# finmath/finmath-lib-cuda-extensions

Measured on AMD Instinct MI355X. Metric: Monte-Carlo path-ops/sec (fused RandomVariable stream), higher is better.
Workload: dtype f32

## Files before the change

finmath-lib-cuda-extensions_amd/host/lmm.hpp:

```cpp
#pragma once
#include <algorithm>
#include <chrono>
#include <cmath>
#include <cstdio>
#include <atomic>
#include <thread>
#include <cstdlib>
#include <functional>
#include <string>
#include <vector>

#include "random_variable.hpp"

namespace fmhost { namespace lmm {


inline const std::vector<double>& atmNormalVolatilities() {
    static const std::vector<double> v = {
        0.00151, 0.00169, 0.0021, 0.00248, 0.00291, 0.00329, 0.00365, 0.004, 0.00437, 0.00466, 0.00527, 0.00571,
        0.00604, 0.00625, 0.0016, 0.00174, 0.00217, 0.00264, 0.00314, 0.00355, 0.00398, 0.00433, 0.00469,
        0.00493, 0.00569, 0.00607, 0.00627, 0.00645, 0.00182, 0.00204, 0.00238, 0.00286, 0.00339, 0.00384,
        0.00424, 0.00456, 0.00488, 0.0052, 0.0059, 0.00623, 0.0064, 0.00654, 0.00205, 0.00235, 0.00272, 0.0032,
        0.00368, 0.00406, 0.00447, 0.00484, 0.00515, 0.00544, 0.00602, 0.00629, 0.0064, 0.00646, 0.00279,
        0.00319, 0.0036, 0.00396, 0.00436, 0.00469, 0.00503, 0.0053, 0.00557, 0.00582, 0.00616, 0.00628,
// ... 71 lines not shown
                for (int p = 0; p < s.numberOfPeriods; ++p) {
                    const double d = curve.df(s.swapTenor[p + 1]);
                    floating += curve.forward(s.swapTenor[p], 0.5) * 0.5 * d; annuity += 0.5 * d;
                }
                s.swaprate = floating / annuity; s.annuity = annuity;
                s.targetVolatility = vols[e * atmTenorYears().size() + k];
                swaptions.push_back(std::move(s));
            }
    }
    int numberOfLibors() const { return timeDiscretization.getNumberOfTimeSteps(); }
};

struct VolatilityModel {
    std::vector<double> grid{ 0.0, 1.0, 2.0, 5.0, 10.0, 20.0, 30.0, 40.0 };
    std::vector<double> parameter = std::vector<double>(64, 0.50 / 100);
    int bin(double x) const { int k = 0; while (k < 7 && grid[(size_t)k] < x - 1e-12) ++k; return k; }
    int parameterIndex(double time, double maturity) const { return bin(time) * 8 + bin(maturity - time); }
    double volatility(double time, double maturity) const { return maturity <= time + 1e-12 ? 0.0 : parameter[(size_t)parameterIndex(time, maturity)]; }
    std::vector<int> activeParameters(const Market& m) const {
        std::vector<char> used(64, 0);
        const auto& td = m.timeDiscretization;
        for (int i = 0; i < td.getNumberOfTimeSteps(); ++i)
            for (int j = i + 1; j < m.numberOfLibors(); ++j) used[(size_t)parameterIndex(td.getTime(i), td.getTime(j))] = 1;
        std::vector<int> idx;
        for (int k = 0; k < 64; ++k) if (used[(size_t)k]) idx.push_back(k);
        return idx;
    }
};


struct Simulation {
    std::vector<std::vector<RV>> libor;
    std::vector<RV> numeraire;
};

struct Backend {
    const RandomVariableFactory* factory = nullptr;
    const BrownianMotion* brownianMotion = nullptr;
    std::function<void()> flush = [] {};
    std::function<void(bool)> hold = [](bool) {};
    std::function<long long()> launches = [] { return 0LL; };
    std::function<std::vector<double>(const std::vector<RV>&)> averages = [](const std::vector<RV>& v) {
        std::vector<double> a; for (const RV& x : v) a.push_back(x->getAverage()); return a; };
    std::function<std::function<std::vector<double>()>(const std::vector<RV>&)> averagesAsync;
    bool expectationsRunPending = false;
    std::function<void(const std::vector<RV>&)> valuesNotNeeded;
    int chunk = 7;
    int stepsPerLaunch = 4;
    std::function<std::vector<std::vector<RV>>(const std::vector<RV>& roots, const std::vector<RV>& leafFrom, const std::vector<std::vector<RV>>& leafTo,
                                               const std::vector<std::vector<double>>* scalars)> clone;
    std::function<std::vector<double>(const std::vector<RV>& roots)> recordedScalars;
    int jacobianBatch = 1;
    bool keepAllStates = false;
    int threads = 1;
};

inline std::vector<Simulation> simulateMany(const Market& m, const std::vector<const VolatilityModel*>& vols, const Backend& be, int lastTimeIndex,
                                            const std::vector<char>* keep = nullptr) {
    const auto& td = m.timeDiscretization;
    const int n = m.numberOfLibors();
    const double delta = m.dt;
    const size_t K = vols.size();
    std::vector<Simulation> sims(K);
    for (Simulation& sim : sims) {
        sim.libor.resize((size_t)lastTimeIndex + 1);
        sim.numeraire.resize((size_t)lastTimeIndex + 1);
        sim.libor[0].resize((size_t)n);
        for (int j = 0; j < n; ++j) sim.libor[0][(size_t)j] = be.factory->createRandomVariable(0.0, m.curve.forward(td.getTime(j), delta));
        sim.numeraire[0] = be.factory->createRandomVariable(0.0, 1.0);
    }
    std::vector<RV> factorSum(K);
    const int S = std::max(1, be.stepsPerLaunch);
    static int cloneChecks = 0;
    for (int i0 = 0; i0 < lastTimeIndex;) {
        int i1 = std::min(i0 + S, lastTimeIndex);
        static const bool endAtKept = std::getenv("FMHIP_LMM_GROUPS_END_AT_KEPT") && std::getenv("FMHIP_LMM_GROUPS_END_AT_KEPT")[0] == '1';
        if (keep && endAtKept) for (int s2 = i0 + 1; s2 < i1; ++s2) if ((*keep)[(size_t)s2]) { i1 = s2; break; }
        const bool cloning = K > 1 && S > 1 && keep && be.clone && i0 >= 2;
        const size_t Krec = cloning ? 1 : K;
        if (S > 1) be.hold(true);
        for (int i = i0; i < i1; ++i) {
            const double t = td.getTime(i), dt = td.getTimeStep(i);
            const RV dW = be.brownianMotion->getBrownianIncrement(i, 0);
            for (size_t k = 0; k < Krec; ++k) {
                auto& cur = sims[k].libor[(size_t)i];
                auto& nxt = sims[k].libor[(size_t)i + 1];
                nxt.resize((size_t)n);
                for (int j = 0; j <= i && j < n; ++j) nxt[(size_t)j] = cur[(size_t)j];
                factorSum[k] = nullptr;
            }
            for (int j0 = i + 1; j0 < n; j0 += be.chunk) {
                const int j1 = std::min(n, j0 + be.chunk);
                for (size_t k = 0; k < Krec; ++k) {
                    auto& cur = sims[k].libor[(size_t)i];
                    auto& nxt = sims[k].libor[(size_t)i + 1];
                    for (int j = j0; j < j1; ++j) {
                        const double lambda = vols[k]->volatility(t, td.getTime(j));
                        const RV& L = cur[(size_t)j];
                        const RV transform = be.factory->createRandomVariable(lambda * delta)->discount(L, delta);
                        factorSum[k] = factorSum[k] ? factorSum[k]->add(transform) : transform;
                        const RV drift = factorSum[k]->mult(lambda);
                        nxt[(size_t)j] = L->addProduct(drift, dt)->addProduct(dW, lambda);
                    }
                }
                if (S == 1 && j1 - j0 == be.chunk) be.flush();
            }
            for (size_t k = 0; k < Krec; ++k)
                sims[k].numeraire[(size_t)i + 1] = sims[k].numeraire[(size_t)i]->accrue(sims[k].libor[(size_t)i][(size_t)i], delta);
            for (size_t k = 0; k < Krec; ++k) factorSum[k] = nullptr;
        }
        if (cloning) {
            std::vector<RV> roots, leafFrom;
            for (int j = i0 + 1; j < n; ++j) roots.push_back(sims[0].libor[(size_t)i1][(size_t)j]);
            for (int i = i0; i < i1; ++i) roots.push_back(sims[0].numeraire[(size_t)i + 1]);
            for (int s2 = i0 + 1; s2 < i1; ++s2)
                if (!keep || (*keep)[(size_t)s2]) for (int j = s2; j < n; ++j) roots.push_back(sims[0].libor[(size_t)s2][(size_t)j]);
            for (int j = i0; j < n; ++j) leafFrom.push_back(sims[0].libor[(size_t)i0][(size_t)j]);
            leafFrom.push_back(sims[0].numeraire[(size_t)i0]);
            auto scalarsOf = [&](const VolatilityModel& vol) {
                std::vector<double> sc;
                for (int i = i0; i < i1; ++i) {
                    const double t = td.getTime(i), dt = td.getTimeStep(i);
                    for (int j = i + 1; j < n; ++j) {
                        const double lambda = vol.volatility(t, td.getTime(j));
                        sc.push_back(delta); sc.push_back(1.0); sc.push_back(lambda * delta); sc.push_back(lambda); sc.push_back(dt); sc.push_back(lambda);
                    }
                    sc.push_back(delta);
                }
                return sc;
            };
            if (cloneChecks < 64 && be.recordedScalars) {
                ++cloneChecks;
                if (be.recordedScalars(roots) != scalarsOf(*vols[0])) throw std::runtime_error("lmm: the scalar list of the replicated Euler steps does not match the recording");
            }
            std::vector<std::vector<RV>> leafTo(K - 1);
            std::vector<std::vector<double>> scalars(K - 1);
            for (size_t k = 1; k < K; ++k) {
                for (int j = i0; j < n; ++j) leafTo[k - 1].push_back(sims[k].libor[(size_t)i0][(size_t)j]);
                leafTo[k - 1].push_back(sims[k].numeraire[(size_t)i0]);
                scalars[k - 1] = scalarsOf(*vols[k]);
            }
            const std::vector<std::vector<RV>> copies = be.clone(roots, leafFrom, leafTo, &scalars);
            for (size_t k = 1; k < K; ++k) {
                auto& nxt = sims[k].libor[(size_t)i1];
                nxt.resize((size_t)n);
                for (int j = 0; j <= i0 && j < n; ++j) nxt[(size_t)j] = sims[k].libor[(size_t)i0][(size_t)j];
                size_t r = 0;
                for (int j = i0 + 1; j < n; ++j) nxt[(size_t)j] = copies[k - 1][r++];
                for (int i = i0; i < i1; ++i) sims[k].numeraire[(size_t)i + 1] = copies[k - 1][r++];
                for (int s2 = i0 + 1; s2 < i1; ++s2)
                    if (!keep || (*keep)[(size_t)s2]) { auto& mid = sims[k].libor[(size_t)s2]; mid.resize((size_t)n); for (int j = s2; j < n; ++j) mid[(size_t)j] = copies[k - 1][r++]; }
            }
        }
        if (keep)
            for (int i = i0; i < i1; ++i)
                if (!(*keep)[(size_t)i])
                    for (size_t k = 0; k < K; ++k) { sims[k].libor[(size_t)i].clear(); sims[k].libor[(size_t)i].shrink_to_fit(); }
        if (S > 1) be.hold(false);
        be.flush();
        i0 = i1;
    }
    return sims;
}

inline Simulation simulate(const Market& m, const VolatilityModel& vol, const Backend& be, int lastTimeIndex) {
    return std::move(simulateMany(m, { &vol }, be, lastTimeIndex)[0]);
}

inline RV swaptionValue(const Market& m, const Simulation& sim, const Swaption& s) {
    const auto& td = m.timeDiscretization;
    const int exerciseIndex = td.getTimeIndex(s.exercise);
    RV value;
    for (int p = s.numberOfPeriods - 1; p >= 0; --p) {
        const int j = td.getTimeIndex(s.swapTenor[(size_t)p]);
        const RV& libor = sim.libor[(size_t)exerciseIndex][(size_t)j];
        const RV payoff = libor->sub(s.swaprate)->mult(s.swapPeriodLength);
        value = (value ? value->add(payoff) : payoff)->discount(libor, s.swapPeriodLength);
    }
    return value->floor(0.0)->div(sim.numeraire[(size_t)exerciseIndex]);
}
inline double bachelierAtmImpliedVolatility(double optionValue, double optionMaturity, double annuity) {
    return optionValue * std::sqrt(2.0 * 3.14159265358979323846) / (annuity * std::sqrt(optionMaturity));
}

struct Valuation { std::vector<double> modelVolatility; double seconds_simulation = 0, seconds_valuation = 0; long long launches_simulation = 0, launches_valuation = 0; };

struct PendingValuations {
    std::vector<std::function<std::vector<double>()>> expectations;
    std::vector<Valuation> out;
};

inline std::vector<Valuation> evaluateManyFinish(const Market& m, PendingValuations& p) {
    for (size_t k = 0; k < p.out.size(); ++k) {
        const std::vector<double> optionValues = p.expectations[k]();
        for (size_t q = 0; q < m.swaptions.size(); ++q)
            p.out[k].modelVolatility.push_back(bachelierAtmImpliedVolatility(optionValues[q], m.swaptions[q].exercise, m.swaptions[q].annuity));
    }
    return std::move(p.out);
}

inline PendingValuations evaluateManyBegin(const Market& m, const std::vector<const VolatilityModel*>& vols, const Backend& be) {
    using clk = std::chrono::steady_clock;
    const size_t K = vols.size();
    PendingValuations pending;
    std::vector<Valuation>& out = pending.out;
    out.resize(K);
    int lastIndex = 0;
    for (const Swaption& s : m.swaptions) lastIndex = std::max(lastIndex, m.timeDiscretization.getTimeIndex(s.exercise));
    const auto t0 = clk::now();
    const long long l0 = be.launches();
    std::vector<char> keep((size_t)lastIndex + 1, 0);
    for (const Swaption& s : m.swaptions) keep[(size_t)m.timeDiscretization.getTimeIndex(s.exercise)] = 1;
    const std::vector<Simulation> sims = simulateMany(m, vols, be, lastIndex, be.keepAllStates ? nullptr : &keep);
    const auto t1 = clk::now();
    const long long l1 = be.launches();
    std::vector<std::vector<RV>> values(K);
    if (K > 1 && be.clone) {
        be.hold(true);
        values[0].reserve(m.swaptions.size());
        for (const Swaption& s : m.swaptions) values[0].push_back(swaptionValue(m, sims[0], s));
        std::vector<RV> leafFrom;
        std::vector<std::vector<RV>> leafTo(K - 1);
        for (int e = 0; e <= lastIndex; ++e) {
            if (!keep[(size_t)e]) continue;
            for (size_t k = 0; k < K; ++k) {
                std::vector<RV>& dst = k == 0 ? leafFrom : leafTo[k - 1];
                for (int j = e; j < m.numberOfLibors(); ++j) dst.push_back(sims[k].libor[(size_t)e][(size_t)j]);
                dst.push_back(sims[k].numeraire[(size_t)e]);
            }
        }
        const std::vector<std::vector<RV>> copies = be.clone(values[0], leafFrom, leafTo, nullptr);
        for (size_t k = 1; k < K; ++k) values[k] = copies[k - 1];
        be.hold(false);
        if (!(be.averagesAsync && be.expectationsRunPending)) be.flush();
    } else
    for (size_t k = 0; k < K; ++k) {
        be.hold(true);
        values[k].reserve(m.swaptions.size());
        for (const Swaption& s : m.swaptions) values[k].push_back(swaptionValue(m, sims[k], s));
        be.hold(false);
        if (!(be.averagesAsync && be.expectationsRunPending)) be.flush();
    }
    if (be.valuesNotNeeded) for (size_t k = 0; k < K; ++k) be.valuesNotNeeded(values[k]);
    for (size_t k = 0; k < K; ++k) {
        if (be.averagesAsync) pending.expectations.push_back(be.averagesAsync(values[k]));
        else { const std::vector<double> now = be.averages(values[k]); pending.expectations.push_back([now] { return now; }); }
    }
    const auto t2 = clk::now();
    for (size_t k = 0; k < K; ++k) {
        out[k].launches_simulation = (l1 - l0) / (long long)K; out[k].launches_valuation = (be.launches() - l1) / (long long)K;
        out[k].seconds_simulation = std::chrono::duration<double>(t1 - t0).count() / (double)K;
        out[k].seconds_valuation = std::chrono::duration<double>(t2 - t1).count() / (double)K;
    }
    return pending;
}

inline std::vector<Valuation> evaluateMany(const Market& m, const std::vector<const VolatilityModel*>& vols, const Backend& be) {
    PendingValuations p = evaluateManyBegin(m, vols, be);
    return evaluateManyFinish(m, p);
}

inline Valuation evaluate(const Market& m, const VolatilityModel& vol, const Backend& be) {
    return std::move(evaluateMany(m, { &vol }, be)[0]);
}


struct CalibrationResult {
    VolatilityModel model; int iterations = 0, evaluations = 0;
    double meanDeviation = 0, rmsDeviation = 0, initialRms = 0, seconds = 0, seconds_simulation = 0, seconds_valuation = 0;
    std::vector<double> modelVolatility;
};

inline bool solveSymmetric(std::vector<double> A, std::vector<double> b, int n, std::vector<double>& x) {
    for (int c = 0; c < n; ++c) {
        int piv = c;
        for (int r = c + 1; r < n; ++r) if (std::fabs(A[(size_t)r * n + c]) > std::fabs(A[(size_t)piv * n + c])) piv = r;
        if (std::fabs(A[(size_t)piv * n + c]) < 1e-300) return false;
        if (piv != c) { for (int k = 0; k < n; ++k) std::swap(A[(size_t)c * n + k], A[(size_t)piv * n + k]); std::swap(b[(size_t)c], b[(size_t)piv]); }
        for (int r = c + 1; r < n; ++r) {
            const double f = A[(size_t)r * n + c] / A[(size_t)c * n + c];
            for (int k = c; k < n; ++k) A[(size_t)r * n + k] -= f * A[(size_t)c * n + k];
            b[(size_t)r] -= f * b[(size_t)c];
        }
    }
    x.assign((size_t)n, 0.0);
    for (int r = n - 1; r >= 0; --r) { double s = b[(size_t)r]; for (int k = r + 1; k < n; ++k) s -= A[(size_t)r * n + k] * x[(size_t)k]; x[(size_t)r] = s / A[(size_t)r * n + r]; }
    return true;
}

inline CalibrationResult calibrate(const Market& m, const Backend& be, int maxIterations = 200, double accuracy = 1e-7,
                                   double lambda = 0.1, double parameterStep = 1e-4, bool verbose = false) {
    using clk = std::chrono::steady_clock;
    const auto start = clk::now();
    CalibrationResult res;
    VolatilityModel vol;
    const std::vector<int> active = vol.activeParameters(m);
    const int np = (int)active.size(), nr = (int)m.swaptions.size();
    auto residuals = [&](const VolatilityModel& v, std::vector<double>& r, std::vector<double>* modelVols) {
        const Valuation val = evaluate(m, v, be);
        res.evaluations++; res.seconds_simulation += val.seconds_simulation; res.seconds_valuation += val.seconds_valuation;
        r.resize((size_t)nr);
        for (int k = 0; k < nr; ++k) r[(size_t)k] = val.modelVolatility[(size_t)k] - m.swaptions[(size_t)k].targetVolatility;
        if (modelVols) *modelVols = val.modelVolatility;
    };
    auto sumsq = [](const std::vector<double>& r) { double s = 0; for (double x : r) s += x * x; return s; };
    std::vector<double> r, rTrial, modelVols;
    residuals(vol, r, &modelVols);
    double err = sumsq(r);
    res.initialRms = std::sqrt(err / nr);
    for (int it = 0; it < maxIterations; ++it) {
        std::vector<double> J((size_t)nr * np);
        struct InFlight { int a0 = 0, a1 = 0; std::vector<VolatilityModel> bumped; PendingValuations pending; bool valid = false; };
        auto collect = [&](InFlight& f) {
            if (!f.valid) return;
            const std::vector<Valuation> vals = evaluateManyFinish(m, f.pending);
            for (int a = f.a0; a < f.a1; ++a) {
                const Valuation& val = vals[(size_t)(a - f.a0)];
                res.evaluations++; res.seconds_simulation += val.seconds_simulation; res.seconds_valuation += val.seconds_valuation;
                for (int k = 0; k < nr; ++k) J[(size_t)k * np + a] = (val.modelVolatility[(size_t)k] - m.swaptions[(size_t)k].targetVolatility - r[(size_t)k]) / parameterStep;
            }
            f.valid = false;
        };
        if (be.threads > 1 && be.jacobianBatch <= 1) {
            const auto tj0 = clk::now();
            std::vector<Valuation> column((size_t)np);
            std::vector<std::string> failures((size_t)be.threads);
            std::atomic<int> next{ 0 };
            std::vector<std::thread> pool;
            for (int t = 0; t < be.threads; ++t)
                pool.emplace_back([&, t] {
                    try {
                        for (int a = next.fetch_add(1); a < np; a = next.fetch_add(1)) {
                            VolatilityModel bumped = vol;
                            bumped.parameter[(size_t)active[(size_t)a]] += parameterStep;
                            column[(size_t)a] = evaluate(m, bumped, be);
                        }
                    } catch (const std::exception& e) { failures[(size_t)t] = e.what(); }
                });
            for (std::thread& th : pool) th.join();
            if (std::getenv("FMHIP_LMM_TIMELINE")) std::fprintf(stderr, "[lmm timeline] iteration %d: %d columns on %d threads, %.3f … %.3f ms\n", it, np, be.threads, std::chrono::duration<double, std::milli>(tj0 - start).count(), std::chrono::duration<double, std::milli>(clk::now() - start).count());
            for (const std::string& f : failures) if (!f.empty()) throw std::runtime_error("a Jacobian column failed: " + f);
            for (int a = 0; a < np; ++a) {
                const Valuation& val = column[(size_t)a];
                res.evaluations++; res.seconds_simulation += val.seconds_simulation; res.seconds_valuation += val.seconds_valuation;
                for (int k = 0; k < nr; ++k) J[(size_t)k * np + a] = (val.modelVolatility[(size_t)k] - m.swaptions[(size_t)k].targetVolatility - r[(size_t)k]) / parameterStep;
            }
        } else {
        InFlight previous;
        for (int a0 = 0; a0 < np; a0 += std::max(1, be.jacobianBatch)) {
            const int a1 = std::min(np, a0 + std::max(1, be.jacobianBatch));
            InFlight current;
            current.a0 = a0; current.a1 = a1;
            current.bumped.assign((size_t)(a1 - a0), vol);
            std::vector<const VolatilityModel*> ptrs;
            for (int a = a0; a < a1; ++a) { current.bumped[(size_t)(a - a0)].parameter[(size_t)active[(size_t)a]] += parameterStep; ptrs.push_back(&current.bumped[(size_t)(a - a0)]); }
            static const bool timeline = std::getenv("FMHIP_LMM_TIMELINE") != nullptr;
            const auto tb0 = clk::now();
            try { current.pending = evaluateManyBegin(m, ptrs, be); current.valid = true; }
            catch (const std::exception& e) {
                if (ptrs.size() == 1 || std::string(e.what()).find("allocation") == std::string::npos) throw;
                if (verbose) std::fprintf(stderr, "  batch of %zu bumps does not fit (%s): evaluating them one at a time\n", ptrs.size(), e.what());
                be.flush();
                collect(previous);
                for (int a = a0; a < a1; ++a) {
                    const Valuation val = evaluate(m, current.bumped[(size_t)(a - a0)], be);
                    res.evaluations++; res.seconds_simulation += val.seconds_simulation; res.seconds_valuation += val.seconds_valuation;
                    for (int k = 0; k < nr; ++k) J[(size_t)k * np + a] = (val.modelVolatility[(size_t)k] - m.swaptions[(size_t)k].targetVolatility - r[(size_t)k]) / parameterStep;
                }
                continue;
            }
            const auto tb1 = clk::now();
            collect(previous);
            if (timeline) std::fprintf(stderr, "[lmm timeline] iteration %d batch from %d: begin %.3f … %.3f ms, previous collected at %.3f ms\n", it, a0,
                                       std::chrono::duration<double, std::milli>(tb0 - start).count(), std::chrono::duration<double, std::milli>(tb1 - start).count(),
                                       std::chrono::duration<double, std::milli>(clk::now() - start).count());
            previous = std::move(current);
        }
        collect(previous);
        }
        std::vector<double> JtJ((size_t)np * np, 0.0), Jtr((size_t)np, 0.0);
        for (int a = 0; a < np; ++a) {
            for (int b = 0; b < np; ++b) { double s = 0; for (int k = 0; k < nr; ++k) s += J[(size_t)k * np + a] * J[(size_t)k * np + b]; JtJ[(size_t)a * np + b] = s; }
            double s = 0; for (int k = 0; k < nr; ++k) s += J[(size_t)k * np + a] * r[(size_t)k]; Jtr[(size_t)a] = -s;
        }
        bool improved = false;
        for (int attempt = 0; attempt < 8 && !improved; ++attempt) {
            std::vector<double> A = JtJ, step;
            for (int a = 0; a < np; ++a) A[(size_t)a * np + a] += lambda * std::max(JtJ[(size_t)a * np + a], 1e-12);
            if (!solveSymmetric(A, Jtr, np, step)) { lambda *= 4; continue; }
            VolatilityModel v = vol;
            for (int a = 0; a < np; ++a) v.parameter[(size_t)active[(size_t)a]] += step[(size_t)a];
            std::vector<double> mv;
            const auto tt0 = clk::now();
            residuals(v, rTrial, &mv);
            static const bool timeline2 = std::getenv("FMHIP_LMM_TIMELINE") != nullptr;
            if (timeline2) std::fprintf(stderr, "[lmm timeline] iteration %d trial %d: %.3f … %.3f ms\n", it, attempt, std::chrono::duration<double, std::milli>(tt0 - start).count(),
                                        std::chrono::duration<double, std::milli>(clk::now() - start).count());
            const double e = sumsq(rTrial);
            if (e < err) { improved = true; const double rel = (err - e) / err; vol = v; r = rTrial; err = e; modelVols = mv; lambda = std::max(lambda / 3.0, 1e-9); if (rel < accuracy) it = maxIterations; }
            else lambda *= 4.0;
        }
        res.iterations++;
        if (verbose) std::fprintf(stderr, "  LM iteration %d: rms %.6e  lambda %.3g  evaluations %d\n", res.iterations, std::sqrt(err / nr), lambda, res.evaluations);
        if (!improved || std::sqrt(err / nr) < accuracy) break;
    }
    res.model = vol; res.modelVolatility = modelVols;
    double sum = 0; for (double x : r) sum += x;
    res.meanDeviation = sum / nr; res.rmsDeviation = std::sqrt(err / nr);
    res.seconds = std::chrono::duration<double>(clk::now() - start).count();
    return res;
}

}}
```

finmath-lib-cuda-extensions_amd/host/lmm_hip_main.cpp:

```cpp
#include <fstream>
#include <thread>
#include <csignal>
#include <execinfo.h>
#include <unistd.h>
#include <rccl/rccl.h>
#include "lmm_main_common.hpp"
#include "hip_backend.hpp"
using namespace fmhost;

static void ncclCheck(ncclResult_t r, const char* what) {
    if (r != ncclSuccess) throw std::runtime_error(std::string(what) + ": " + ncclGetErrorString(r));
}

static void fatalSignal(int sig) {
    void* frames[64];
    const int n = backtrace(frames, 64);
    const char msg[] = "lmm_hip: fatal signal, call stack:\n";
    (void)!write(2, msg, sizeof msg - 1);
    backtrace_symbols_fd(frames, n, 2);
    signal(sig, SIG_DFL);
    raise(sig);
}

int main(int argc, char** argv) {
    if (std::getenv("FMHIP_BACKTRACE")) { signal(SIGABRT, fatalSignal); signal(SIGSEGV, fatalSignal); signal(SIGBUS, fatalSignal); }
    const lmm::Options o = lmm::parseOptions(argc, argv);
    try {
        if (!o.devices.empty()) check(fmhip_init_devices(o.devices.data(), (int)o.devices.size()));
        else check(fmhip_init(-1));
        check(fmhip_set_fusion(1, nullptr));
        RandomVariableHipFactory factory;
        lmm::Market m;
        const int64_t pathOffset = o.pathOffset + (int64_t)o.rank * o.paths;
        BrownianMotionHip philox(m.timeDiscretization, 1, o.paths, o.seed, pathOffset);
        BrownianMotionFromMersenneRandomNumbers mersenne(m.timeDiscretization, 1, o.paths, (int)o.seed, &factory);
        if (o.brownian == "mersenne" && o.world > 1) throw std::runtime_error("--brownian mersenne is a sequential stream: not available with --world > 1 (mersenne-device is)");
        BrownianMotionFromMersenneRandomNumbersHip mersenneDevice(m.timeDiscretization, 1, o.paths, (int)o.seed, pathOffset);
        lmm::Backend be = makeHipBackend(&factory, (o.brownian == "mersenne") ? static_cast<const BrownianMotion*>(&mersenne)
                                                 : (o.brownian == "mersenne-device") ? static_cast<const BrownianMotion*>(&mersenneDevice) : &philox,
                                         o.chunk, o.stepsPerLaunch, o.jacobianBatch);

        if (o.finmathLike) {
            be.flush = [] {}; be.hold = [](bool) {}; be.clone = nullptr; be.recordedScalars = nullptr; be.averagesAsync = nullptr; be.expectationsRunPending = false;
            be.averages = [](const std::vector<RV>& v) { std::vector<double> a; for (const RV& x : v) a.push_back(x->getAverage()); return a; };
            be.jacobianBatch = 1; be.stepsPerLaunch = 1; be.chunk = 1 << 30; be.keepAllStates = true;
            if (o.threads > 1) {
                if (!o.devices.empty() || o.world > 1) throw std::runtime_error("--threads: one device, one process");
                check(fmhip_set_thread_engines(1, nullptr));
                be.threads = o.threads;
            }
        } else if (o.threads > 1) throw std::runtime_error("--threads belongs to --finmath-like (the native driver batches its Jacobian columns instead)");
        if (o.releaseLagMs > 0.0 || o.releaseLagBytes > 0) ReleaseLag::instance().start(o.releaseLagMs, (size_t)o.releaseLagBytes);
        ncclComm_t comm = nullptr;
        std::vector<std::pair<double*, hipEvent_t>> sparePinned;
        fmhip_vec sums = 0;
        long long collectives = 0;
        double collective_seconds = 0.0;
        if (o.world > 1 || !o.ncclIdFile.empty()) {
            if (o.ncclIdFile.empty()) throw std::runtime_error("--world needs --nccl-id-file");
            struct IdFile { uint64_t magic, nonce; ncclUniqueId id; } rec{};
            const uint64_t MAGIC = 0x464d4e43434c4944ull;
            if (o.rank == 0) {
                std::remove(o.ncclIdFile.c_str());
                rec.magic = MAGIC; rec.nonce = (uint64_t)o.ncclNonce;
                ncclCheck(ncclGetUniqueId(&rec.id), "ncclGetUniqueId");
                { std::ofstream f(o.ncclIdFile + ".tmp", std::ios::binary); f.write((const char*)&rec, sizeof rec); }
                std::rename((o.ncclIdFile + ".tmp").c_str(), o.ncclIdFile.c_str());
            } else {
                for (int tries = 0; ; ++tries) {
                    std::ifstream f(o.ncclIdFile, std::ios::binary);
                    if (f && f.read((char*)&rec, sizeof rec) && f.gcount() == (std::streamsize)sizeof rec && rec.magic == MAGIC && rec.nonce == (uint64_t)o.ncclNonce) break;
                    if (tries > 6000) throw std::runtime_error("timed out waiting for " + o.ncclIdFile);
                    std::this_thread::sleep_for(std::chrono::milliseconds(10));
                }
            }
            const ncclUniqueId id = rec.id;
            ncclCheck(ncclCommInitRank(&comm, o.world, id, o.rank), "ncclCommInitRank");
            if (o.rank == 0) std::remove(o.ncclIdFile.c_str());
            const int count = (int)m.swaptions.size();
            check(fmhip_vec_create_uninitialized((int64_t)count * 8 * o.world, &sums));
            void* stream = nullptr; check(fmhip_get_stream(&stream));
            const int64_t totalPaths = (int64_t)o.world * o.paths;
            const int world = o.world, rank = o.rank;
            struct Flight {
                fmhip_vec dev = 0; double* host = nullptr; hipEvent_t ev = nullptr;
                std::vector<std::pair<double*, hipEvent_t>>* spare = nullptr;
                ~Flight() { if (dev) fmhip_vec_release(dev); if (host && ev && spare) spare->push_back({ host, ev }); }
            };
            std::vector<std::pair<double*, hipEvent_t>>* const spare = &sparePinned;
            { const char* e = std::getenv("FMHIP_LMM_SHARDED_FROM_LAUNCHES"); be.expectationsRunPending = !(e && e[0] == '0'); }
            be.averagesAsync = [=, &collectives, &collective_seconds](const std::vector<RV>& v) -> std::function<std::vector<double>()> {
                std::vector<fmhip_vec> h;
                for (const RV& x : v) {
                    auto p = dynamic_cast<const RandomVariableHip*>(x.get());
                    if (!p || p->isDeterministic()) throw std::runtime_error("sharded expectation of a non-device value");
                    h.push_back(p->deviceVector().handle());
                }
                if ((int)h.size() != count) throw std::runtime_error("sharded expectation: unexpected product count");
                auto f = std::make_shared<Flight>();
                const size_t doubles = (size_t)count * 4 * (size_t)world;
                check(fmhip_vec_create_uninitialized((int64_t)doubles * 2, &f->dev));
                f->spare = spare;
                if (!spare->empty()) { f->host = spare->back().first; f->ev = spare->back().second; spare->pop_back(); }
                else if (hipHostMalloc((void**)&f->host, doubles * 8, hipHostMallocDefault) != hipSuccess || hipEventCreateWithFlags(&f->ev, hipEventDisableTiming) != hipSuccess)
                    throw std::runtime_error("pinned memory / event for a sharded expectation");
                void* dev = nullptr; check(fmhip_vec_device_ptr(f->dev, &dev));
                double* all = (double*)dev;
                check(fmhip_reduce_moments_batch_device(h.data(), count, nullptr, all + (size_t)rank * count * 4));
                ncclCheck(ncclAllGather(all + (size_t)rank * count * 4, all, (size_t)count * 4, ncclDouble, comm, (hipStream_t)stream), "ncclAllGather");
                if (hipMemcpyAsync(f->host, all, doubles * 8, hipMemcpyDeviceToHost, (hipStream_t)stream) != hipSuccess || hipEventRecord(f->ev, (hipStream_t)stream) != hipSuccess)
                    throw std::runtime_error("enqueueing the read-back of a sharded expectation");
                ++collectives;
// ... 100 lines not shown
```

finmath-lib-cuda-extensions_amd/host/lmm_main_common.hpp:

```cpp
#pragma once
#include <vector>
#include <cstdlib>
#include <cstring>
#include <string>
#include "lmm.hpp"

namespace fmhost { namespace lmm {

struct Options {
    int64_t paths = 10000; int64_t seed = 31415; int maxIterations = 200; std::string mode = "calibrate"; bool verbose = false;
    int64_t pathOffset = 0; int evaluations = 1;
    int warmupEvaluations = 0;
    int world = 1, rank = 0; std::string ncclIdFile; long long ncclNonce = 0;
    std::vector<int> devices;
    int chunk = 0;
    int stepsPerLaunch = 0;
    int jacobianBatch = 0;
    std::string brownian = "philox";
    int threads = 1;
    double releaseLagMs = 0.0;
    long long releaseLagBytes = 0;
    bool finmathLike = false;
    bool profile = false;
};
inline Options parseOptions(int argc, char** argv) {
    Options o;
    for (int i = 1; i < argc; ++i) {
        const std::string a = argv[i];
        auto next = [&]() -> const char* { if (i + 1 >= argc) { std::fprintf(stderr, "missing value for %s\n", a.c_str()); std::exit(2); } return argv[++i]; };
        if (a == "--paths") o.paths = std::atoll(next());
        else if (a == "--seed") o.seed = std::atoll(next());
        else if (a == "--max-iterations") o.maxIterations = std::atoi(next());
        else if (a == "--mode") o.mode = next();
        else if (a == "--evaluations") o.evaluations = std::atoi(next());
        else if (a == "--warmup-evaluations") o.warmupEvaluations = std::atoi(next());
        else if (a == "--path-offset") o.pathOffset = std::atoll(next());
        else if (a == "--world") o.world = std::atoi(next());
        else if (a == "--devices") { std::string list = next(); size_t p0 = 0; while (p0 <= list.size()) { const size_t q = list.find(',', p0); o.devices.push_back(std::atoi(list.substr(p0, q == std::string::npos ? std::string::npos : q - p0).c_str())); if (q == std::string::npos) break; p0 = q + 1; } }
        else if (a == "--rank") o.rank = std::atoi(next());
        else if (a == "--nccl-id-file") o.ncclIdFile = next();
        else if (a == "--nccl-nonce") o.ncclNonce = std::atoll(next());
        else if (a == "--profile") o.profile = true;
        else if (a == "--finmath-like") o.finmathLike = true;
        else if (a == "--threads") o.threads = std::atoi(next());
        else if (a == "--release-lag") o.releaseLagMs = std::atof(next());
        else if (a == "--release-lag-bytes") o.releaseLagBytes = std::atoll(next());
        else if (a == "--brownian") o.brownian = next();
        else if (a == "--jacobian-batch") o.jacobianBatch = std::atoi(next());
        else if (a == "--chunk") o.chunk = std::atoi(next());
        else if (a == "--steps-per-launch") o.stepsPerLaunch = std::atoi(next());
        else if (a == "--verbose") o.verbose = true;
        else { std::fprintf(stderr, "unknown option %s\n", a.c_str()); std::exit(2); }
    }
    return o;
}

inline void runAndReport(const Options& o, const Backend& be, const char* backendName, const std::function<std::string()>& extraJson) {
    Market m;
    if (o.mode == "evaluate") {
        VolatilityModel vol;
        Valuation v;
        double sim = 0, val = 0;
        const int K = std::max(1, o.jacobianBatch);
        for (int k = 0; k < o.evaluations; k += K) {
            const int kk = std::min(K, o.evaluations - k);
            const std::vector<Valuation> vs = evaluateMany(m, std::vector<const VolatilityModel*>((size_t)kk, &vol), be);
            for (const Valuation& x : vs) { sim += x.seconds_simulation; val += x.seconds_valuation; }
            v = vs.back();
        }
        std::printf("{\"backend\": \"%s\", \"mode\": \"evaluate\", \"paths\": %lld, \"swaptions\": %zu, \"evaluations\": %d, "
                    "\"seconds_simulation_per_evaluation\": %.6f, \"seconds_valuation_per_evaluation\": %.6f, \"launches_simulation\": %lld, \"launches_valuation\": %lld%s, \"model_volatility\": [",
                    backendName, (long long)o.paths, m.swaptions.size(), o.evaluations, sim / o.evaluations, val / o.evaluations, v.launches_simulation, v.launches_valuation, extraJson().c_str());
        for (size_t k = 0; k < v.modelVolatility.size(); ++k) std::printf("%s%.17g", k ? ", " : "", v.modelVolatility[k]);
        std::printf("]}\n");
        return;
    }
    const CalibrationResult r = calibrate(m, be, o.maxIterations, 1e-7, 0.1, 1e-4, o.verbose);
    std::printf("{\"backend\": \"%s\", \"mode\": \"calibrate\", \"paths\": %lld, \"swaptions\": %zu, \"active_parameters\": %zu, "
                "\"iterations\": %d, \"evaluations\": %d, \"seconds\": %.4f, \"seconds_simulation\": %.4f, \"seconds_valuation\": %.4f, "
                "\"initial_rms\": %.6e, \"rms_deviation\": %.6e, \"mean_deviation\": %.6e%s, \"parameters\": [",
                backendName, (long long)o.paths, m.swaptions.size(), VolatilityModel().activeParameters(m).size(), r.iterations, r.evaluations,
                r.seconds, r.seconds_simulation, r.seconds_valuation, r.initialRms, r.rmsDeviation, r.meanDeviation, extraJson().c_str());
    for (size_t k = 0; k < r.model.parameter.size(); ++k) std::printf("%s%.17g", k ? ", " : "", r.model.parameter[k]);
    std::printf("]}\n");
}

}}
```

Measured before the change: 4324 billion.

## Reuse base simulation prefix and skip unaffected products in Jacobian bumps

For each bumped volatility parameter, the Jacobian evaluation now copies the base simulation's states up to the first time step that reads the bumped parameter. It re-simulates only from that step on and revalues only swaptions whose exercise comes after it. Columns whose parameter never affects any exercise are given zero derivatives without any evaluation. The change adds bookkeeping for the base states (extra kept time indices, a stored trial simulation) and is disabled in finmath-like and multi-rank modes.

```diff
diff --git a/finmath-lib-cuda-extensions_amd/host/lmm.hpp b/finmath-lib-cuda-extensions_amd/host/lmm.hpp
--- a/finmath-lib-cuda-extensions_amd/host/lmm.hpp
+++ b/finmath-lib-cuda-extensions_amd/host/lmm.hpp
@@ -147,11 +147,34 @@
     std::function<std::vector<double>(const std::vector<RV>& roots)> recordedScalars;
     int jacobianBatch = 1;
     bool keepAllStates = false;
+    bool reuseBase = true;
+    bool productSubsets = true;
     int threads = 1;
 };
 
+inline std::vector<std::pair<int, int>> stepGroups(const Backend& be, int lastTimeIndex, const std::vector<char>* keep) {
+    static const bool endAtKept = std::getenv("FMHIP_LMM_GROUPS_END_AT_KEPT") && std::getenv("FMHIP_LMM_GROUPS_END_AT_KEPT")[0] == '1';
+    const int S = std::max(1, be.stepsPerLaunch);
+    std::vector<std::pair<int, int>> groups;
+    for (int i0 = 0; i0 < lastTimeIndex;) {
+        int i1 = std::min(i0 + S, lastTimeIndex);
+        if (keep && endAtKept) for (int s2 = i0 + 1; s2 < i1; ++s2) if ((*keep)[(size_t)s2]) { i1 = s2; break; }
+        groups.push_back({ i0, i1 });
+        i0 = i1;
+    }
+    return groups;
+}
+
+inline int firstStepReading(const Market& m, const VolatilityModel& vol, int parameter, int lastTimeIndex) {
+    const auto& td = m.timeDiscretization;
+    for (int i = 0; i < lastTimeIndex; ++i)
+        for (int j = i + 1; j < m.numberOfLibors(); ++j) if (vol.parameterIndex(td.getTime(i), td.getTime(j)) == parameter) return i;
+    return -1;
+}
+
 inline std::vector<Simulation> simulateMany(const Market& m, const std::vector<const VolatilityModel*>& vols, const Backend& be, int lastTimeIndex,
-                                            const std::vector<char>* keep = nullptr) {
+                                            const std::vector<char>* keep = nullptr, const Simulation* base = nullptr, const std::vector<int>* start = nullptr,
+                                            long long* groupsFromBase = nullptr) {
     const auto& td = m.timeDiscretization;
     const int n = m.numberOfLibors();
     const double delta = m.dt;
@@ -167,17 +190,29 @@
     std::vector<RV> factorSum(K);
     const int S = std::max(1, be.stepsPerLaunch);
     static int cloneChecks = 0;
-    for (int i0 = 0; i0 < lastTimeIndex;) {
-        int i1 = std::min(i0 + S, lastTimeIndex);
-        static const bool endAtKept = std::getenv("FMHIP_LMM_GROUPS_END_AT_KEPT") && std::getenv("FMHIP_LMM_GROUPS_END_AT_KEPT")[0] == '1';
-        if (keep && endAtKept) for (int s2 = i0 + 1; s2 < i1; ++s2) if ((*keep)[(size_t)s2]) { i1 = s2; break; }
-        const bool cloning = K > 1 && S > 1 && keep && be.clone && i0 >= 2;
-        const size_t Krec = cloning ? 1 : K;
+    if (base && (!start || start->size() != K)) throw std::runtime_error("lmm: a base simulation needs a start per parameter set");
+    for (const std::pair<int, int>& group : stepGroups(be, lastTimeIndex, keep)) {
+        const int i0 = group.first, i1 = group.second;
+        std::vector<size_t> act;
+        for (size_t k = 0; k < K; ++k) {
+            if (!base || (*start)[k] < i1) { act.push_back(k); continue; }
+            for (int i = i0 + 1; i <= i1; ++i) {
+                sims[k].numeraire[(size_t)i] = base->numeraire[(size_t)i];
+                if (!keep || (*keep)[(size_t)i] || i == (*start)[k]) {
+                    if (base->libor[(size_t)i].size() != (size_t)n) throw std::runtime_error("lmm: the base simulation does not hold the state at time index " + std::to_string(i));
+                    sims[k].libor[(size_t)i] = base->libor[(size_t)i];
+                }
+            }
+            if (groupsFromBase) ++*groupsFromBase;
+        }
+        const bool cloning = act.size() > 1 && S > 1 && keep && be.clone && i0 >= 2;
+        const std::vector<size_t> rec = cloning ? std::vector<size_t>{ act[0] } : act;
+        const size_t k0 = act.empty() ? 0 : act[0];
         if (S > 1) be.hold(true);
-        for (int i = i0; i < i1; ++i) {
+        for (int i = i0; i < i1 && !act.empty(); ++i) {
             const double t = td.getTime(i), dt = td.getTimeStep(i);
             const RV dW = be.brownianMotion->getBrownianIncrement(i, 0);
-            for (size_t k = 0; k < Krec; ++k) {
+            for (const size_t k : rec) {
                 auto& cur = sims[k].libor[(size_t)i];
                 auto& nxt = sims[k].libor[(size_t)i + 1];
                 nxt.resize((size_t)n);
@@ -186,7 +221,7 @@
             }
             for (int j0 = i + 1; j0 < n; j0 += be.chunk) {
                 const int j1 = std::min(n, j0 + be.chunk);
-                for (size_t k = 0; k < Krec; ++k) {
+                for (const size_t k : rec) {
                     auto& cur = sims[k].libor[(size_t)i];
                     auto& nxt = sims[k].libor[(size_t)i + 1];
                     for (int j = j0; j < j1; ++j) {
@@ -200,18 +235,18 @@
                 }
                 if (S == 1 && j1 - j0 == be.chunk) be.flush();
             }
-            for (size_t k = 0; k < Krec; ++k)
+            for (const size_t k : rec)
                 sims[k].numeraire[(size_t)i + 1] = sims[k].numeraire[(size_t)i]->accrue(sims[k].libor[(size_t)i][(size_t)i], delta);
-            for (size_t k = 0; k < Krec; ++k) factorSum[k] = nullptr;
+            for (const size_t k : rec) factorSum[k] = nullptr;
         }
         if (cloning) {
             std::vector<RV> roots, leafFrom;
-            for (int j = i0 + 1; j < n; ++j) roots.push_back(sims[0].libor[(size_t)i1][(size_t)j]);
-            for (int i = i0; i < i1; ++i) roots.push_back(sims[0].numeraire[(size_t)i + 1]);
+            for (int j = i0 + 1; j < n; ++j) roots.push_back(sims[k0].libor[(size_t)i1][(size_t)j]);
+            for (int i = i0; i < i1; ++i) roots.push_back(sims[k0].numeraire[(size_t)i + 1]);
             for (int s2 = i0 + 1; s2 < i1; ++s2)
-                if (!keep || (*keep)[(size_t)s2]) for (int j = s2; j < n; ++j) roots.push_back(sims[0].libor[(size_t)s2][(size_t)j]);
-            for (int j = i0; j < n; ++j) leafFrom.push_back(sims[0].libor[(size_t)i0][(size_t)j]);
-            leafFrom.push_back(sims[0].numeraire[(size_t)i0]);
+                if (!keep || (*keep)[(size_t)s2]) for (int j = s2; j < n; ++j) roots.push_back(sims[k0].libor[(size_t)s2][(size_t)j]);
+            for (int j = i0; j < n; ++j) leafFrom.push_back(sims[k0].libor[(size_t)i0][(size_t)j]);
+            leafFrom.push_back(sims[k0].numeraire[(size_t)i0]);
             auto scalarsOf = [&](const VolatilityModel& vol) {
                 std::vector<double> sc;
                 for (int i = i0; i < i1; ++i) {
@@ -226,25 +261,29 @@
             };
             if (cloneChecks < 64 && be.recordedScalars) {
                 ++cloneChecks;
-                if (be.recordedScalars(roots) != scalarsOf(*vols[0])) throw std::runtime_error("lmm: the scalar list of the replicated Euler steps does not match the recording");
-            }
-            std::vector<std::vector<RV>> leafTo(K - 1);
-            std::vector<std::vector<double>> scalars(K - 1);
-            for (size_t k = 1; k < K; ++k) {
-                for (int j = i0; j < n; ++j) leafTo[k - 1].push_back(sims[k].libor[(size_t)i0][(size_t)j]);
-                leafTo[k - 1].push_back(sims[k].numeraire[(size_t)i0]);
-                scalars[k - 1] = scalarsOf(*vols[k]);
+                if (be.recordedScalars(roots) != scalarsOf(*vols[k0])) throw std::runtime_error("lmm: the scalar list of the replicated Euler steps does not match the recording");
+            }
+            const size_t C = act.size() - 1;
+            std::vector<std::vector<RV>> leafTo(C);
+            std::vector<std::vector<double>> scalars(C);
+            for (size_t c = 0; c < C; ++c) {
+                const size_t k = act[c + 1];
+                if (sims[k].libor[(size_t)i0].size() != (size_t)n) throw std::runtime_error("lmm: a parameter set has no state to start from at time index " + std::to_string(i0));
+                for (int j = i0; j < n; ++j) leafTo[c].push_back(sims[k].libor[(size_t)i0][(size_t)j]);
+                leafTo[c].push_back(sims[k].numeraire[(size_t)i0]);
+                scalars[c] = scalarsOf(*vols[k]);
             }
             const std::vector<std::vector<RV>> copies = be.clone(roots, leafFrom, leafTo, &scalars);
-            for (size_t k = 1; k < K; ++k) {
+            for (size_t c = 0; c < C; ++c) {
+                const size_t k = act[c + 1];
                 auto& nxt = sims[k].libor[(size_t)i1];
                 nxt.resize((size_t)n);
                 for (int j = 0; j <= i0 && j < n; ++j) nxt[(size_t)j] = sims[k].libor[(size_t)i0][(size_t)j];
                 size_t r = 0;
-                for (int j = i0 + 1; j < n; ++j) nxt[(size_t)j] = copies[k - 1][r++];
-                for (int i = i0; i < i1; ++i) sims[k].numeraire[(size_t)i + 1] = copies[k - 1][r++];
+                for (int j = i0 + 1; j < n; ++j) nxt[(size_t)j] = copies[c][r++];
+                for (int i = i0; i < i1; ++i) sims[k].numeraire[(size_t)i + 1] = copies[c][r++];
                 for (int s2 = i0 + 1; s2 < i1; ++s2)
-                    if (!keep || (*keep)[(size_t)s2]) { auto& mid = sims[k].libor[(size_t)s2]; mid.resize((size_t)n); for (int j = s2; j < n; ++j) mid[(size_t)j] = copies[k - 1][r++]; }
+                    if (!keep || (*keep)[(size_t)s2]) { auto& mid = sims[k].libor[(size_t)s2]; mid.resize((size_t)n); for (int j = s2; j < n; ++j) mid[(size_t)j] = copies[c][r++]; }
             }
         }
         if (keep)
@@ -253,7 +292,6 @@
                     for (size_t k = 0; k < K; ++k) { sims[k].libor[(size_t)i].clear(); sims[k].libor[(size_t)i].shrink_to_fit(); }
         if (S > 1) be.hold(false);
         be.flush();
-        i0 = i1;
     }
     return sims;
 }
@@ -280,59 +318,108 @@
 
 struct Valuation { std::vector<double> modelVolatility; double seconds_simulation = 0, seconds_valuation = 0; long long launches_simulation = 0, launches_valuation = 0; };
 
+struct BaseReuse {
+    const std::vector<char>* keepAlso = nullptr;
+    std::vector<Simulation>* simulationsOut = nullptr;
+    const Simulation* base = nullptr;
+    const std::vector<double>* baseModelVolatility = nullptr;
+    std::vector<int> start;
+};
+
 struct PendingValuations {
     std::vector<std::function<std::vector<double>()>> expectations;
+    std::vector<std::vector<int>> products;
+    std::vector<double> baseModelVolatility;
+    long long groupsFromBase = 0, productsFromBase = 0;
     std::vector<Valuation> out;
 };
 
 inline std::vector<Valuation> evaluateManyFinish(const Market& m, PendingValuations& p) {
     for (size_t k = 0; k < p.out.size(); ++k) {
         const std::vector<double> optionValues = p.expectations[k]();
-        for (size_t q = 0; q < m.swaptions.size(); ++q)
-            p.out[k].modelVolatility.push_back(bachelierAtmImpliedVolatility(optionValues[q], m.swaptions[q].exercise, m.swaptions[q].annuity));
+        if (optionValues.size() != p.products[k].size()) throw std::runtime_error("lmm: a back end returned another number of expectations than it was asked for");
+        p.out[k].modelVolatility = p.baseModelVolatility;
+        p.out[k].modelVolatility.resize(m.swaptions.size(), 0.0);
+        for (size_t r = 0; r < p.products[k].size(); ++r) {
+            const size_t q = (size_t)p.products[k][r];
+            p.out[k].modelVolatility[q] = bachelierAtmImpliedVolatility(optionValues[r], m.swaptions[q].exercise, m.swaptions[q].annuity);
+        }
     }
     return std::move(p.out);
 }
 
-inline PendingValuations evaluateManyBegin(const Market& m, const std::vector<const VolatilityModel*>& vols, const Backend& be) {
+inline int lastExerciseIndex(const Market& m) {
+    int lastIndex = 0;
+    for (const Swaption& s : m.swaptions) lastIndex = std::max(lastIndex, m.timeDiscretization.getTimeIndex(s.exercise));
+    return lastIndex;
+}
+inline std::vector<char> exerciseIndices(const Market& m) {
+    std::vector<char> keep((size_t)lastExerciseIndex(m) + 1, 0);
+    for (const Swaption& s : m.swaptions) keep[(size_t)m.timeDiscretization.getTimeIndex(s.exercise)] = 1;
+    return keep;
+}
+
+inline PendingValuations evaluateManyBegin(const Market& m, const std::vector<const VolatilityModel*>& vols, const Backend& be, const BaseReuse* reuse = nullptr) {
     using clk = std::chrono::steady_clock;
     const size_t K = vols.size();
     PendingValuations pending;
     std::vector<Valuation>& out = pending.out;
     out.resize(K);
-    int lastIndex = 0;
-    for (const Swaption& s : m.swaptions) lastIndex = std::max(lastIndex, m.timeDiscretization.getTimeIndex(s.exercise));
+    const int lastIndex = lastExerciseIndex(m);
     const auto t0 = clk::now();
     const long long l0 = be.launches();
-    std::vector<char> keep((size_t)lastIndex + 1, 0);
-    for (const Swaption& s : m.swaptions) keep[(size_t)m.timeDiscretization.getTimeIndex(s.exercise)] = 1;
-    const std::vector<Simulation> sims = simulateMany(m, vols, be, lastIndex, be.keepAllStates ? nullptr : &keep);
+    const std::vector<char> exercise = exerciseIndices(m);
+    std::vector<char> keep = exercise;
+    if (reuse && reuse->keepAlso) for (size_t i = 0; i < keep.size() && i < reuse->keepAlso->size(); ++i) keep[i] |= (*reuse->keepAlso)[i];
+    const Simulation* base = reuse ? reuse->base : nullptr;
+    if (base && (reuse->start.size() != K || !reuse->baseModelVolatility)) throw std::runtime_error("lmm: a base simulation needs a start per parameter set and the base's model volatilities");
+    std::vector<Simulation> sims = simulateMany(m, vols, be, lastIndex, be.keepAllStates ? nullptr : &keep, base, base ? &reuse->start : nullptr, &pending.groupsFromBase);
     const auto t1 = clk::now();
     const long long l1 = be.launches();
+    const bool subsets = base && be.productSubsets;
+    auto exerciseIndexOf = [&](size_t q) { return m.timeDiscretization.getTimeIndex(m.swaptions[q].exercise); };
+    pending.products.resize(K);
+    for (size_t k = 0; k < K; ++k)
+        for (size_t q = 0; q < m.swaptions.size(); ++q)
+            if (!subsets || exerciseIndexOf(q) > reuse->start[k]) pending.products[k].push_back((int)q);
+            else ++pending.productsFromBase;
+    if (subsets) pending.baseModelVolatility = *reuse->baseModelVolatility;
     std::vector<std::vector<RV>> values(K);
+    auto record = [&](size_t k) {
+        values[k].reserve(pending.products[k].size());
+        for (const int q : pending.products[k]) values[k].push_back(swaptionValue(m, sims[k], m.swaptions[(size_t)q]));
+    };
     if (K > 1 && be.clone) {
         be.hold(true);
-        values[0].reserve(m.swaptions.size());
-        for (const Swaption& s : m.swaptions) values[0].push_back(swaptionValue(m, sims[0], s));
-        std::vector<RV> leafFrom;
-        std::vector<std::vector<RV>> leafTo(K - 1);
-        for (int e = 0; e <= lastIndex; ++e) {
-            if (!keep[(size_t)e]) continue;
-            for (size_t k = 0; k < K; ++k) {
-                std::vector<RV>& dst = k == 0 ? leafFrom : leafTo[k - 1];
-                for (int j = e; j < m.numberOfLibors(); ++j) dst.push_back(sims[k].libor[(size_t)e][(size_t)j]);
-                dst.push_back(sims[k].numeraire[(size_t)e]);
-            }
-        }
-        const std::vector<std::vector<RV>> copies = be.clone(values[0], leafFrom, leafTo, nullptr);
-        for (size_t k = 1; k < K; ++k) values[k] = copies[k - 1];
+        std::vector<char> done(K, 0);
+        for (size_t k0 = 0; k0 < K; ++k0) {
+            if (done[k0]) continue;
+            std::vector<size_t> members;
+            for (size_t k = k0; k < K; ++k) if (!done[k] && (!subsets || reuse->start[k] == reuse->start[k0])) { members.push_back(k); done[k] = 1; }
+            record(k0);
+            if (members.size() == 1 || values[k0].empty()) continue;
+            int firstOwn = 0;
+            if (base) { firstOwn = lastIndex; for (const size_t k : members) firstOwn = std::min(firstOwn, reuse->start[k]); }
+            std::vector<RV> leafFrom;
+            std::vector<std::vector<RV>> leafTo(members.size() - 1);
+            for (int e = 0; e <= lastIndex; ++e) {
+                if (!exercise[(size_t)e] || (base && e <= firstOwn)) continue;
+                for (size_t c = 0; c < members.size(); ++c) {
+                    std::vector<RV>& dst = c == 0 ? leafFrom : leafTo[c - 1];
+                    const Simulation& sim = sims[members[c]];
+                    for (int j = e; j < m.numberOfLibors(); ++j) dst.push_back(sim.libor[(size_t)e][(size_t)j]);
+                    dst.push_back(sim.numeraire[(size_t)e]);
+                }
+            }
+            const std::vector<std::vector<RV>> copies = be.clone(values[k0], leafFrom, leafTo, nullptr);
+            for (size_t c = 1; c < members.size(); ++c) values[members[c]] = copies[c - 1];
+        }
         be.hold(false);
         if (!(be.averagesAsync && be.expectationsRunPending)) be.flush();
     } else
     for (size_t k = 0; k < K; ++k) {
         be.hold(true);
-        values[k].reserve(m.swaptions.size());
-        for (const Swaption& s : m.swaptions) values[k].push_back(swaptionValue(m, sims[k], s));
+        record(k);
         be.hold(false);
         if (!(be.averagesAsync && be.expectationsRunPending)) be.flush();
     }
@@ -347,6 +434,7 @@
         out[k].seconds_simulation = std::chrono::duration<double>(t1 - t0).count() / (double)K;
         out[k].seconds_valuation = std::chrono::duration<double>(t2 - t1).count() / (double)K;
     }
+    if (reuse && reuse->simulationsOut) *reuse->simulationsOut = std::move(sims);
     return pending;
 }
 
@@ -364,6 +452,7 @@
     VolatilityModel model; int iterations = 0, evaluations = 0;
     double meanDeviation = 0, rmsDeviation = 0, initialRms = 0, seconds = 0, seconds_simulation = 0, seconds_valuation = 0;
     std::vector<double> modelVolatility;
+    int columnsWithoutEffect = 0; long long groupsFromBase = 0, productsFromBase = 0;
 };
 
 inline bool solveSymmetric(std::vector<double> A, std::vector<double> b, int n, std::vector<double>& x) {
@@ -391,8 +480,32 @@
     VolatilityModel vol;
     const std::vector<int> active = vol.activeParameters(m);
     const int np = (int)active.size(), nr = (int)m.swaptions.size();
-    auto residuals = [&](const VolatilityModel& v, std::vector<double>& r, std::vector<double>* modelVols) {
-        const Valuation val = evaluate(m, v, be);
+    static const bool reuseSwitch = !(std::getenv("FMHIP_LMM_REUSE_BASE") && std::getenv("FMHIP_LMM_REUSE_BASE")[0] == '0');
+    const bool reuse = reuseSwitch && be.reuseBase && !be.keepAllStates && be.threads <= 1;
+    const int lastIndex = lastExerciseIndex(m);
+    std::vector<int> columnStart((size_t)np, 0);
+    std::vector<char> keepStarts((size_t)lastIndex + 1, 0);
+    long long groupCount = 0;
+    if (reuse) {
+        const std::vector<char> exercise = exerciseIndices(m);
+        const std::vector<std::pair<int, int>> groups = stepGroups(be, lastIndex, &exercise);
+        groupCount = (long long)groups.size();
+        for (int a = 0; a < np; ++a) {
+            const int first = firstStepReading(m, vol, active[(size_t)a], lastIndex);
+            columnStart[(size_t)a] = lastIndex;
+            if (first < 0) { res.columnsWithoutEffect++; continue; }
+            for (const auto& g : groups) if (g.first <= first && first < g.second) columnStart[(size_t)a] = g.first;
+            keepStarts[(size_t)columnStart[(size_t)a]] = 1;
+        }
+    }
+    Simulation baseSimulation, trialSimulation;
+    auto residuals = [&](const VolatilityModel& v, std::vector<double>& r, std::vector<double>* modelVols, Simulation* simulation) {
+        BaseReuse hold;
+        std::vector<Simulation> sims;
+        hold.keepAlso = &keepStarts; hold.simulationsOut = &sims;
+        PendingValuations p = evaluateManyBegin(m, { &v }, be, reuse ? &hold : nullptr);
+        const Valuation val = std::move(evaluateManyFinish(m, p)[0]);
+        if (reuse && simulation) *simulation = std::move(sims[0]);
         res.evaluations++; res.seconds_simulation += val.seconds_simulation; res.seconds_valuation += val.seconds_valuation;
         r.resize((size_t)nr);
         for (int k = 0; k < nr; ++k) r[(size_t)k] = val.modelVolatility[(size_t)k] - m.swaptions[(size_t)k].targetVolatility;
@@ -400,17 +513,18 @@
     };
     auto sumsq = [](const std::vector<double>& r) { double s = 0; for (double x : r) s += x * x; return s; };
     std::vector<double> r, rTrial, modelVols;
-    residuals(vol, r, &modelVols);
+    residuals(vol, r, &modelVols, &baseSimulation);
     double err = sumsq(r);
     res.initialRms = std::sqrt(err / nr);
     for (int it = 0; it < maxIterations; ++it) {
         std::vector<double> J((size_t)nr * np);
-        struct InFlight { int a0 = 0, a1 = 0; std::vector<VolatilityModel> bumped; PendingValuations pending; bool valid = false; };
+        struct InFlight { std::vector<int> columns; std::vector<VolatilityModel> bumped; PendingValuations pending; bool valid = false; };
         auto collect = [&](InFlight& f) {
             if (!f.valid) return;
             const std::vector<Valuation> vals = evaluateManyFinish(m, f.pending);
-            for (int a = f.a0; a < f.a1; ++a) {
-                const Valuation& val = vals[(size_t)(a - f.a0)];
+            for (size_t c = 0; c < f.columns.size(); ++c) {
+                const int a = f.columns[c];
+                const Valuation& val = vals[c];
                 res.evaluations++; res.seconds_simulation += val.seconds_simulation; res.seconds_valuation += val.seconds_valuation;
                 for (int k = 0; k < nr; ++k) J[(size_t)k * np + a] = (val.modelVolatility[(size_t)k] - m.swaptions[(size_t)k].targetVolatility - r[(size_t)k]) / parameterStep;
             }
@@ -442,23 +556,42 @@
             }
         } else {
         InFlight previous;
-        for (int a0 = 0; a0 < np; a0 += std::max(1, be.jacobianBatch)) {
-            const int a1 = std::min(np, a0 + std::max(1, be.jacobianBatch));
+        std::vector<int> columns;
+        for (int a = 0; a < np; ++a) {
+            if (reuse && be.productSubsets && columnStart[(size_t)a] >= lastIndex) {
+                res.evaluations++; res.productsFromBase += nr; res.groupsFromBase += groupCount;
+                for (int k = 0; k < nr; ++k) J[(size_t)k * np + a] = 0.0;
+            } else columns.push_back(a);
+        }
+        const int batch = std::max(1, be.jacobianBatch);
+        for (size_t c0 = 0; c0 < columns.size(); c0 += (size_t)batch) {
+            const size_t c1 = std::min(columns.size(), c0 + (size_t)batch);
+            const int a0 = columns[c0];
             InFlight current;
-            current.a0 = a0; current.a1 = a1;
-            current.bumped.assign((size_t)(a1 - a0), vol);
+            current.columns.assign(columns.begin() + (long)c0, columns.begin() + (long)c1);
+            current.bumped.assign(c1 - c0, vol);
             std::vector<const VolatilityModel*> ptrs;
-            for (int a = a0; a < a1; ++a) { current.bumped[(size_t)(a - a0)].parameter[(size_t)active[(size_t)a]] += parameterStep; ptrs.push_back(&current.bumped[(size_t)(a - a0)]); }
+            BaseReuse from;
+            from.keepAlso = &keepStarts; from.base = &baseSimulation; from.baseModelVolatility = &modelVols;
+            for (size_t c = c0; c < c1; ++c) {
+                const int a = columns[c];
+                current.bumped[c - c0].parameter[(size_t)active[(size_t)a]] += parameterStep; ptrs.push_back(&current.bumped[c - c0]);
+                from.start.push_back(columnStart[(size_t)a]);
+            }
             static const bool timeline = std::getenv("FMHIP_LMM_TIMELINE") != nullptr;
             const auto tb0 = clk::now();
-            try { current.pending = evaluateManyBegin(m, ptrs, be); current.valid = true; }
+            try {
+                current.pending = evaluateManyBegin(m, ptrs, be, reuse ? &from : nullptr); current.valid = true;
+                res.groupsFromBase += current.pending.groupsFromBase; res.productsFromBase += current.pending.productsFromBase;
+            }
             catch (const std::exception& e) {
                 if (ptrs.size() == 1 || std::string(e.what()).find("allocation") == std::string::npos) throw;
                 if (verbose) std::fprintf(stderr, "  batch of %zu bumps does not fit (%s): evaluating them one at a time\n", ptrs.size(), e.what());
                 be.flush();
                 collect(previous);
-                for (int a = a0; a < a1; ++a) {
-                    const Valuation val = evaluate(m, current.bumped[(size_t)(a - a0)], be);
+                for (size_t c = c0; c < c1; ++c) {
+                    const int a = columns[c];
+                    const Valuation val = evaluate(m, current.bumped[c - c0], be);
                     res.evaluations++; res.seconds_simulation += val.seconds_simulation; res.seconds_valuation += val.seconds_valuation;
                     for (int k = 0; k < nr; ++k) J[(size_t)k * np + a] = (val.modelVolatility[(size_t)k] - m.swaptions[(size_t)k].targetVolatility - r[(size_t)k]) / parameterStep;
                 }
@@ -487,11 +620,13 @@
             for (int a = 0; a < np; ++a) v.parameter[(size_t)active[(size_t)a]] += step[(size_t)a];
             std::vector<double> mv;
             const auto tt0 = clk::now();
-            residuals(v, rTrial, &mv);
+            residuals(v, rTrial, &mv, &trialSimulation);
             static const bool timeline2 = std::getenv("FMHIP_LMM_TIMELINE") != nullptr;
             if (timeline2) std::fprintf(stderr, "[lmm timeline] iteration %d trial %d: %.3f … %.3f ms\n", it, attempt, std::chrono::duration<double, std::milli>(tt0 - start).count(),
                                         std::chrono::duration<double, std::milli>(clk::now() - start).count());
             const double e = sumsq(rTrial);
+            if (e < err) baseSimulation = std::move(trialSimulation);
+            trialSimulation = Simulation();
             if (e < err) { improved = true; const double rel = (err - e) / err; vol = v; r = rTrial; err = e; modelVols = mv; lambda = std::max(lambda / 3.0, 1e-9); if (rel < accuracy) it = maxIterations; }
             else lambda *= 4.0;
         }
diff --git a/finmath-lib-cuda-extensions_amd/host/lmm_hip_main.cpp b/finmath-lib-cuda-extensions_amd/host/lmm_hip_main.cpp
--- a/finmath-lib-cuda-extensions_amd/host/lmm_hip_main.cpp
+++ b/finmath-lib-cuda-extensions_amd/host/lmm_hip_main.cpp
@@ -43,7 +43,7 @@
         if (o.finmathLike) {
             be.flush = [] {}; be.hold = [](bool) {}; be.clone = nullptr; be.recordedScalars = nullptr; be.averagesAsync = nullptr; be.expectationsRunPending = false;
             be.averages = [](const std::vector<RV>& v) { std::vector<double> a; for (const RV& x : v) a.push_back(x->getAverage()); return a; };
-            be.jacobianBatch = 1; be.stepsPerLaunch = 1; be.chunk = 1 << 30; be.keepAllStates = true;
+            be.jacobianBatch = 1; be.stepsPerLaunch = 1; be.chunk = 1 << 30; be.keepAllStates = true; be.reuseBase = false;
             if (o.threads > 1) {
                 if (!o.devices.empty() || o.world > 1) throw std::runtime_error("--threads: one device, one process");
                 check(fmhip_set_thread_engines(1, nullptr));
@@ -58,6 +58,7 @@
         double collective_seconds = 0.0;
         if (o.world > 1 || !o.ncclIdFile.empty()) {
             if (o.ncclIdFile.empty()) throw std::runtime_error("--world needs --nccl-id-file");
+            be.productSubsets = false;
             struct IdFile { uint64_t magic, nonce; ncclUniqueId id; } rec{};
             const uint64_t MAGIC = 0x464d4e43434c4944ull;
             if (o.rank == 0) {
diff --git a/finmath-lib-cuda-extensions_amd/host/lmm_main_common.hpp b/finmath-lib-cuda-extensions_amd/host/lmm_main_common.hpp
--- a/finmath-lib-cuda-extensions_amd/host/lmm_main_common.hpp
+++ b/finmath-lib-cuda-extensions_amd/host/lmm_main_common.hpp
@@ -55,8 +55,14 @@
     return o;
 }
 
-inline void runAndReport(const Options& o, const Backend& be, const char* backendName, const std::function<std::string()>& extraJson) {
+inline void runAndReport(const Options& o, const Backend& backend, const char* backendName, const std::function<std::string()>& extraJson) {
     Market m;
+    Backend be = backend;
+    if (!o.finmathLike) {
+        if (o.chunk > 0) be.chunk = o.chunk;
+        if (o.stepsPerLaunch > 0) be.stepsPerLaunch = o.stepsPerLaunch;
+        if (o.jacobianBatch > 0) be.jacobianBatch = o.jacobianBatch;
+    }
     if (o.mode == "evaluate") {
         VolatilityModel vol;
         Valuation v;
@@ -78,9 +84,11 @@
     const CalibrationResult r = calibrate(m, be, o.maxIterations, 1e-7, 0.1, 1e-4, o.verbose);
     std::printf("{\"backend\": \"%s\", \"mode\": \"calibrate\", \"paths\": %lld, \"swaptions\": %zu, \"active_parameters\": %zu, "
                 "\"iterations\": %d, \"evaluations\": %d, \"seconds\": %.4f, \"seconds_simulation\": %.4f, \"seconds_valuation\": %.4f, "
-                "\"initial_rms\": %.6e, \"rms_deviation\": %.6e, \"mean_deviation\": %.6e%s, \"parameters\": [",
+                "\"initial_rms\": %.6e, \"rms_deviation\": %.6e, \"mean_deviation\": %.6e, "
+                "\"columns_without_effect\": %d, \"simulation_groups_taken_from_base\": %lld, \"products_taken_from_base\": %lld%s, \"parameters\": [",
                 backendName, (long long)o.paths, m.swaptions.size(), VolatilityModel().activeParameters(m).size(), r.iterations, r.evaluations,
-                r.seconds, r.seconds_simulation, r.seconds_valuation, r.initialRms, r.rmsDeviation, r.meanDeviation, extraJson().c_str());
+                r.seconds, r.seconds_simulation, r.seconds_valuation, r.initialRms, r.rmsDeviation, r.meanDeviation,
+                r.columnsWithoutEffect, r.groupsFromBase, r.productsFromBase, extraJson().c_str());
     for (size_t k = 0; k < r.model.parameter.size(); ++k) std::printf("%s%.17g", k ? ", " : "", r.model.parameter[k]);
     std::printf("]}\n");
 }
```

Measured after the change: 4266 billion. 0.986x the previous value.
